# jl6017/AutoURDF

Hardware: AMD Instinct MI355X
Metric: registered frames/sec (N=4096 pts, K=20 clusters) (higher is better)
Workload: dtype f32

## Files before the change

autourdf_amd/csrc/train_backward.hip:

```cpp
#include <cmath>
#include <cstddef>
#include <cstring>
#include "train_dev.h"

namespace creg {

__device__ __forceinline__ TrainState advance_state(const TrainState& S, float loss, const Hyper& hy, double bc1, float bc2_sqrt) {
    TrainState N = S;
    const bool improved = loss < S.min_loss;
    N.last_loss = loss;
    N.epochs_run = S.epochs_run + 1;
    const int count = improved ? 0 : S.count + 1;
    N.min_loss = improved ? loss : S.min_loss;
    N.best_epoch = improved ? S.epochs_run : S.best_epoch;
    N.count = count;
    N.stopped = (!improved && count > hy.stop) ? 1 : S.stopped;
    if (!N.stopped) {
        N.step = S.step + 1;
        N.step_size = (float)(S.lr / bc1);
        N.bc2_sqrt = bc2_sqrt;
        const double cur = (double)loss;
        if (cur < S.sched_best * (1.0 - 1e-4)) { N.sched_best = cur; N.sched_bad = 0; }
        else N.sched_bad = S.sched_bad + 1;
        if (N.sched_bad > hy.patience) {
            const double nl = fmax(S.lr * (double)hy.factor, 0.0);
            if (S.lr - nl > 1e-8) N.lr = nl;
            N.sched_bad = 0;
        }
    }
    return N;
}

constexpr int GC_QMAX = 3;
__device__ __forceinline__ void gradc_role(const Dims& D, const Ws& W, int epoch, int nbx, int nby, int k) {
    __shared__ float red[4][14];
    __shared__ float s_loss;
    __shared__ float s_go[16];
    const int tid = threadIdx.x, lane = tid & 63, wv = tid >> 6;
    const TrainState S = W.state[epoch & 1];
    const int b0 = W.off[k], e0 = W.off[k + 1];
    const Hyper hy = *W.hyper;
    float a = tid < nbx ? W.lossp_x[tid] : 0.f, b = tid < nby ? W.lossp_y[tid] : 0.f;
    const float m2v = W.m2[16 * k + (tid & 15)];
    float sv[16];
#pragma unroll
    for (int i = 0; i < 16; ++i) sv[i] = W.head_save[16 * k + i];
    const float* h2cur = (epoch & 1) ? W.h2[1] : W.h2[0];
    float w3v[GC_QMAX][8], h2v[GC_QMAX];
#pragma unroll
    for (int q = 0; q < GC_QMAX; ++q) {
        const int o = min(q * 256 + tid, D.H2 - 1);
        const bool isA = o < D.HA;
        const float* Pc = (epoch & 1) ? W.P1 : W.P;
        const float* wb = isA ? Pc + D.oW3A + o : Pc + D.oW3B + (o - D.HA);
        const int stride = isA ? D.HA : D.HB, nj = isA ? D.OA : D.OB;
#pragma unroll
        for (int j = 0; j < 8; ++j) w3v[q][j] = wb[(size_t)min(j, nj - 1) * stride];
        h2v[q] = h2cur[(size_t)k * D.H2 + o];
    }
    asm volatile("" :: "v"(a), "v"(b), "v"(m2v), "v"(sv[0]), "v"(sv[1]), "v"(sv[2]), "v"(sv[3]), "v"(sv[4]), "v"(sv[5]), "v"(sv[6]), "v"(sv[7]),
                 "v"(sv[8]), "v"(sv[9]), "v"(sv[10]), "v"(sv[11]), "v"(sv[12]), "v"(sv[13]), "v"(sv[14]), "v"(sv[15]), "v"(b0), "v"(e0), "v"(hy.lr));
#pragma unroll
    for (int q = 0; q < GC_QMAX; ++q)
        asm volatile("" :: "v"(h2v[q]), "v"(w3v[q][0]), "v"(w3v[q][1]), "v"(w3v[q][2]), "v"(w3v[q][3]), "v"(w3v[q][4]), "v"(w3v[q][5]), "v"(w3v[q][6]),
                     "v"(w3v[q][7]));
    if (S.stopped) {
        if (k == 0 && tid == 0) {
            TrainState E = S; E.stopped = 1;
            W.state[(epoch + 1) & 1] = E;
        }
        return;
    }
    const int n_first = min(b0 + tid, D.NP - 1);
    const float4 p_first = W.pts4[n_first];
    const int4 c_first = W.cnt4[n_first];
    const int s_first = W.sgn_x[n_first];
    const float4 pr_first = W.pred4[n_first];
    for (int i = tid + 256; i < nbx; i += 256) a += W.lossp_x[i];
    for (int i = tid + 256; i < nby; i += 256) b += W.lossp_y[i];
    a = wave_sum_fast(a); b = wave_sum_fast(b);
    if (lane == 0) { red[wv][0] = a; red[wv][1] = b; }
    __syncthreads();
    if (tid == 0) {
        const float sa = ((red[0][0] + red[1][0]) + red[2][0]) + red[3][0];
        const float sb = ((red[0][1] + red[1][1]) + red[2][1]) + red[3][1];
        s_loss = sa / (float)D.NP + sb / (float)D.NT;
    }
    __syncthreads();
    const float loss = s_loss;
    TrainState N = advance_state(S, loss, hy, S.next_bc1, S.next_bc2s);
    const bool improved = loss < S.min_loss;
    if (improved) {
        for (int n = b0 + tid; n < e0; n += 256) {
            const float4 p = (n == b0 + tid) ? pr_first : W.pred4[n];
            W.best_pred[3 * (size_t)n] = p.x; W.best_pred[3 * (size_t)n + 1] = p.y; W.best_pred[3 * (size_t)n + 2] = p.z;
        }
        if (tid < 16) W.best_m[16 * k + tid] = m2v;
    }
    if (k == 0 && tid == 0) {
        N.next_bc1 = W.bc1[min(N.step + 1, D.epochs)];
        N.next_bc2s = W.bc2s[min(N.step + 1, D.epochs)];
        W.state[(epoch + 1) & 1] = N;
        W.loss_hist[S.epochs_run] = loss;
        W.lr_hist[S.epochs_run] = (float)S.lr;
        W.result[0] = N.min_loss; W.result[1] = (float)N.epochs_run; W.result[2] = (float)N.lr; W.result[3] = (float)N.best_epoch;
    }
    if (N.stopped) return;
    const float gx = 1.0f / (float)D.NP, gy = 1.0f / (float)D.NT;
    float acc[12];
#pragma unroll
    for (int i = 0; i < 12; ++i) acc[i] = 0.f;
    for (int n = b0 + tid; n < e0; n += 256) {
        const bool first = n == b0 + tid;
        const float4 p = first ? p_first : W.pts4[n];
        const int4 c = first ? c_first : W.cnt4[n];
        const int sb = first ? s_first : W.sgn_x[n];
        const float g[3] = {((sb & 1) ? gx : -gx) + gy * (float)c.x, ((sb & 2) ? gx : -gx) + gy * (float)c.y,
                            ((sb & 4) ? gx : -gx) + gy * (float)c.z};
#pragma unroll
        for (int q = 0; q < 3; ++q) {
            acc[4 * q] = fmaf(g[q], p.x, acc[4 * q]); acc[4 * q + 1] = fmaf(g[q], p.y, acc[4 * q + 1]);
            acc[4 * q + 2] = fmaf(g[q], p.z, acc[4 * q + 2]); acc[4 * q + 3] += g[q];
        }
    }
    __syncthreads();
#pragma unroll
    for (int i = 0; i < 12; ++i) { const float r = wave_sum_fast(acc[i]); if (lane == 0) red[wv][i] = r; }
    __syncthreads();
    if (tid == 0) {
        float G12[12];
        for (int i = 0; i < 12; ++i) G12[i] = ((red[0][i] + red[1][i]) + red[2][i]) + red[3][i];
        for (int i = 0; i < 16; ++i) W.gm2[16 * k + i] = i < 12 ? G12[i] : 0.f;
        const float G[9] = {G12[0], G12[1], G12[2], G12[4], G12[5], G12[6], G12[8], G12[9], G12[10]};
        const float gt[3] = {G12[3], G12[7], G12[11]};
        float go[16];
        for (int i = 0; i < 16; ++i) go[i] = 0.f;
        if (D.rot == ROT_6D) {
            go[0] = gt[0]; go[1] = gt[1]; go[2] = gt[2];
            rot6d_to_matrix_vjp(sv, G, go + 4);
        } else if (D.rot == ROT_RPY) {
            go[0] = gt[0]; go[1] = gt[1]; go[2] = gt[2];
            float ge[3];
            euler_xyz_to_matrix_vjp(sv, G, ge);
            for (int i = 0; i < 3; ++i) go[4 + i] = ge[i] * (1.f - sv[4 + i] * sv[4 + i]);
        } else if (D.rot == ROT_Q) {
            go[0] = gt[0]; go[1] = gt[1]; go[2] = gt[2];
            float gu[4];
            quat_to_matrix_vjp(sv, G, gu);
            const float nrm = sv[4];
            if (nrm > 1e-12f) {
                const float dot = sv[0] * gu[0] + sv[1] * gu[1] + sv[2] * gu[2] + sv[3] * gu[3];
#pragma unroll
                for (int i = 0; i < 4; ++i) go[4 + i] = (gu[i] - sv[i] * dot) / nrm;
            } else {
#pragma unroll
                for (int i = 0; i < 4; ++i) go[4 + i] = gu[i] / 1e-12f;
            }
        } else {
            float gdq[8];
            dq_to_se3_vjp(sv, G, gt, gdq);
            for (int i = 0; i < 8; ++i) go[4 + i] = gdq[i];
        }
        for (int i = 0; i < 12; ++i) { W.g_out[16 * k + i] = go[i]; s_go[i] = go[i]; }
    }
    __syncthreads();
#pragma unroll
    for (int q = 0; q < GC_QMAX; ++q) {
        const int o = q * 256 + tid;
        if (o < D.H2) {
            const bool isA = o < D.HA;
            const int nj = isA ? D.OA : D.OB, gofs = isA ? 0 : 4;
            float sum = 0.f;
#pragma unroll
            for (int j = 0; j < 8; ++j) if (j < nj) sum = fmaf(s_go[gofs + j], w3v[q][j], sum);
            W.g_h2[(size_t)k * D.H2 + o] = sum * act_grad(h2v[q], D.slope);
        }
    }
}

__global__ __launch_bounds__(256) void k_gradc(Dims D, Ws W0, int epoch, int nbx, int nby, size_t bstride) {
    asm volatile("" :: "s"(W0.P), "s"(W0.P1), "s"(W0.h2[0]), "s"(W0.h2[1]), "s"(W0.head_save), "s"(W0.m2), "s"(W0.gm2), "s"(W0.pts4), "s"(W0.pred4),
                 "s"(W0.sgn_x), "s"(W0.cnt4), "s"(W0.lossp_x), "s"(W0.lossp_y), "s"(W0.g_out), "s"(W0.g_h2), "s"(W0.state), "s"(W0.bc1), "s"(W0.bc2s),
                 "s"(W0.best_m), "s"(W0.best_pred), "s"(W0.loss_hist), "s"(W0.lr_hist), "s"(W0.result), "s"(W0.off), "s"(W0.hyper),
                 "s"(D.rot), "s"(D.K), "s"(D.H2), "s"(D.HA), "s"(D.HB), "s"(D.OA), "s"(D.OB), "s"(D.NP), "s"(D.NT), "s"(D.epochs), "s"(D.slope),
                 "s"(D.oW3A), "s"(D.oW3B), "s"(epoch), "s"(nbx), "s"(nby), "s"(bstride));
    const Ws W = ws_shift(W0, blockIdx.z * bstride);
    gradc_role(D, W, epoch, nbx, nby, blockIdx.x);
}

__device__ __forceinline__ float adam_value(float p, float& mm, float& vv, float g, float step_size, float bc2_sqrt) {
    const float b1w = (float)(1.0 - 0.9), b2 = 0.999f, b2w = (float)(1.0 - 0.999);
    mm = mm + b1w * (g - mm);
    vv = vv * b2 + (b2w * g) * g;
    const float denom = sqrtf(vv) / bc2_sqrt + 1e-8f;
    return p + (-step_size * mm) / denom;
}

#ifdef CREG_BD_STAMPS
struct BdStamps {
    unsigned long long first[256], endB[256], endD[256], startB[256], startD[256];
    unsigned long long phase[2][8], blocks[2];
    int armed;
};
__device__ BdStamps g_bd_st;
#endif
constexpr int BD_THREADS = 512;
constexpr int B2_THREADS = BD_THREADS;
constexpr int B2_WAVES = B2_THREADS / 64;
constexpr int B2_CB = 16;
constexpr int B2_RB = 32;
__host__ __device__ inline int b2_smem_floats(int K, int IN, int H2) {
    return B2_WAVES * B2_RB * B2_CB + K * IN + 2 * K * B2_CB + H2 * B2_CB;
}
__device__ __forceinline__ float row_sum16(float v) {
    CREG_DPP_STEP(v, 0xB1, 0xF);
    CREG_DPP_STEP(v, 0x4E, 0xF);
    CREG_DPP_STEP(v, 0x141, 0xF);
    CREG_DPP_STEP(v, 0x140, 0xF);
    return v;
}

template <int KW, bool X>
__device__ __forceinline__ void bwd2_role(const Dims& D, const Ws& W, int epoch, int blk, float* sh, unsigned long long bd_entry) {
    constexpr int NS = KW / 4;
    constexpr bool V4 = KW % 16 == 0;
    constexpr int NA = V4 ? NS / 4 : NS;
    float* red = sh;
    float* encs = red + B2_WAVES * B2_RB * B2_CB;
    float* gxs = encs + D.K * D.IN;
    float* xt = gxs + D.K * B2_CB;
    float* w2s = xt + D.K * B2_CB;
    const int tid = threadIdx.x, lane = tid & 63, wv = tid >> 6, lj = lane & 15, kk = lane >> 4;
    __builtin_amdgcn_s_waitcnt(0x0F70);
    const int c0 = blk * B2_CB, par = epoch & 1;
    const float* x1cur = par ? W.x1[1] : W.x1[0];
    float* x1next = par ? W.x1[0] : W.x1[1];
    const float* Pc = par ? W.P1 : W.P;
    float* Pn = par ? W.P : W.P1;
    BD_T0
    {
        const float* src = Pc + D.oW2 + (size_t)(wv * KW + (lane >> 2)) * D.H + c0 + 4 * (lane & 3);
        float* dst = w2s + wv * KW * B2_CB;
#pragma unroll
        for (int i = 0; i < KW; i += 16)
            if (i + (lane >> 2) < KW)
                __builtin_amdgcn_global_load_lds((const __attribute__((address_space(1))) void*)(src + (size_t)i * D.H),
                                                 (__attribute__((address_space(3))) void*)(dst + i * B2_CB), 16, 0, 0);
    }
    const float* gbase = W.g_h2 + wv * KW + (V4 ? 4 * kk : kk);
    auto load_a = [&](int row, float* dst) {
        const float* g = gbase + (size_t)min(row, D.K - 1) * D.H2;
#pragma unroll
        for (int q = 0; q < NA; ++q) {
            if constexpr (V4) { const float4 v = *(const float4*)(g + 16 * q); dst[4 * q] = v.x; dst[4 * q + 1] = v.y; dst[4 * q + 2] = v.z; dst[4 * q + 3] = v.w; }
            else dst[q] = g[4 * q];
        }
    };
    float a0[NS], a1[NS];
    const bool two0 = D.K > 16;
    load_a(lj, a0);
    if (two0) load_a(16 + lj, a1);
    const int half = tid >> 8, t2 = tid & 255, row = t2 >> 4, i4 = t2 & 15, hu = c0 + row;
    const bool ain = 4 * i4 < D.IN;
    const int ei = min(4 * i4, D.IN - 4);
    const size_t wi = (size_t)D.oW1 + (size_t)hu * D.IN + ei;
    float4 pw = *(const float4*)(Pc + wi), pm = *(const float4*)(W.AM + wi), pv = *(const float4*)(W.AV + wi);
    const bool ain2 = X && 64 + 4 * i4 < D.IN;
    const int ei2 = min(64 + 4 * i4, D.IN - 4);
    const size_t wi2 = (size_t)D.oW1 + (size_t)hu * D.IN + ei2;
    float4 pw2, pm2, pv2;
    if constexpr (X) { pw2 = *(const float4*)(Pc + wi2); pm2 = *(const float4*)(W.AM + wi2); pv2 = *(const float4*)(W.AV + wi2); }
    float pb = Pc[D.ob1 + hu], mb = W.AM[D.ob1 + hu], vb = W.AV[D.ob1 + hu];
    float xv0 = x1cur[(size_t)min(tid >> 4, D.K - 1) * D.H + c0 + (tid & 15)];
    {
        const int n = D.K * D.IN / 4;
        constexpr int NPC = 8;
#pragma unroll
        for (int c = 0; c < NPC; ++c) {
            const int i = c * B2_THREADS + tid;
            if (i < n)
                __builtin_amdgcn_global_load_lds((const __attribute__((address_space(1))) void*)((const float4*)W.enc + i),
                                                 (__attribute__((address_space(3))) void*)((float4*)encs + c * B2_THREADS + (tid & ~63)), 16, 0, 0);
        }
    }
    __builtin_amdgcn_sched_barrier(0);
    const TrainState S = W.state[(epoch + 1) & 1];
    const bool live = !S.stopped;
    __builtin_amdgcn_sched_barrier(0);
    BD_T
    stage_wait();
    float wb[NS];
#pragma unroll
    for (int s = 0; s < NS; ++s) {
        const int o = V4 ? 16 * (s >> 2) + 4 * kk + (s & 3) : 4 * s + kk;
        wb[s] = w2s[(wv * KW + o) * B2_CB + lj];
    }
    for (int r0 = 0; r0 < D.K; r0 += B2_RB) {
        const int nr = min(B2_RB, D.K - r0);
        const bool two = nr > 16;
        float xv = xv0;
        if (r0) {
            load_a(r0 + lj, a0);
            if (two) load_a(r0 + 16 + lj, a1);
            xv = x1cur[(size_t)min(r0 + (tid >> 4), D.K - 1) * D.H + c0 + (tid & 15)];
        }
        f32x4 acc0 = {0.f, 0.f, 0.f, 0.f}, acc1 = {0.f, 0.f, 0.f, 0.f};
        if (two) {
#pragma unroll
            for (int s = 0; s < NS; ++s) {
                acc0 = __builtin_amdgcn_mfma_f32_16x16x4f32(a0[s], wb[s], acc0, 0, 0, 0);
                acc1 = __builtin_amdgcn_mfma_f32_16x16x4f32(a1[s], wb[s], acc1, 0, 0, 0);
            }
        } else {
#pragma unroll
            for (int s = 0; s < NS; ++s) acc0 = __builtin_amdgcn_mfma_f32_16x16x4f32(a0[s], wb[s], acc0, 0, 0, 0);
        }
        if (r0) __syncthreads();
        {
            float* o = red + (wv * B2_RB + 4 * kk) * B2_CB + lj;
#pragma unroll
            for (int v = 0; v < 4; ++v) { o[v * B2_CB] = acc0[v]; if (two) o[(16 + v) * B2_CB] = acc1[v]; }
        }
        stage_wait();
        __syncthreads();
        if (r0 == 0) { BD_T }
        if (!live) return;
        if (tid < nr * B2_CB) {
            float sum = red[tid];
#pragma unroll
            for (int w2 = 1; w2 < B2_WAVES; ++w2) sum += red[w2 * B2_RB * B2_CB + tid];
            gxs[r0 * B2_CB + tid] = sum * act_grad(xv, D.slope);
        }
    }
    __syncthreads();
    BD_T
    float4 ag = make_float4(0.f, 0.f, 0.f, 0.f), ag2 = make_float4(0.f, 0.f, 0.f, 0.f);
    float gsum = 0.f;
    for (int r = 0; r < D.K; ++r) {
        const float g = gxs[r * B2_CB + row];
        const float4 e = *(const float4*)(encs + r * D.IN + ei);
        ag.x = fmaf(g, e.x, ag.x); ag.y = fmaf(g, e.y, ag.y); ag.z = fmaf(g, e.z, ag.z); ag.w = fmaf(g, e.w, ag.w);
        if constexpr (X) {
            const float4 e2 = *(const float4*)(encs + r * D.IN + ei2);
            ag2.x = fmaf(g, e2.x, ag2.x); ag2.y = fmaf(g, e2.y, ag2.y); ag2.z = fmaf(g, e2.z, ag2.z); ag2.w = fmaf(g, e2.w, ag2.w);
        }
        gsum += g;
    }
    float4 nw;
    nw.x = adam_value(pw.x, pm.x, pv.x, ag.x, S.step_size, S.bc2_sqrt);
    nw.y = adam_value(pw.y, pm.y, pv.y, ag.y, S.step_size, S.bc2_sqrt);
    nw.z = adam_value(pw.z, pm.z, pv.z, ag.z, S.step_size, S.bc2_sqrt);
    nw.w = adam_value(pw.w, pm.w, pv.w, ag.w, S.step_size, S.bc2_sqrt);
    float4 nw2 = make_float4(0.f, 0.f, 0.f, 0.f);
    if constexpr (X) {
        nw2.x = adam_value(pw2.x, pm2.x, pv2.x, ag2.x, S.step_size, S.bc2_sqrt);
        nw2.y = adam_value(pw2.y, pm2.y, pv2.y, ag2.y, S.step_size, S.bc2_sqrt);
        nw2.z = adam_value(pw2.z, pm2.z, pv2.z, ag2.z, S.step_size, S.bc2_sqrt);
        nw2.w = adam_value(pw2.w, pm2.w, pv2.w, ag2.w, S.step_size, S.bc2_sqrt);
    }
    pb = adam_value(pb, mb, vb, gsum, S.step_size, S.bc2_sqrt);
    if (live && half == 0) {
        if (ain) { st4_wt(Pn, wi, nw); st4_wt(W.AM, wi, pm); st4_wt(W.AV, wi, pv); }
        if constexpr (X) if (ain2) { st4_wt(Pn, wi2, nw2); st4_wt(W.AM, wi2, pm2); st4_wt(W.AV, wi2, pv2); }
        if (i4 == 0) { Pn[D.ob1 + hu] = pb; W.AM[D.ob1 + hu] = mb; W.AV[D.ob1 + hu] = vb; }
    }
    BD_T
    for (int r = half; r < D.K; r += 2) {
        const float4 e = *(const float4*)(encs + r * D.IN + ei);
        float v = ain ? fmaf(nw.w, e.w, fmaf(nw.z, e.z, fmaf(nw.y, e.y, nw.x * e.x))) : 0.f;
        if constexpr (X) {
            const float4 e2 = *(const float4*)(encs + r * D.IN + ei2);
            if (ain2) v = fmaf(nw2.w, e2.w, fmaf(nw2.z, e2.z, fmaf(nw2.y, e2.y, fmaf(nw2.x, e2.x, v))));
        }
        v = row_sum16(v) + pb;
        if (i4 == 0) xt[r * B2_CB + row] = act_f(v, D.slope);
    }
    __syncthreads();
    if (live)
        for (int t = tid; t < D.K * (B2_CB / 2); t += B2_THREADS) {
            const int r = t >> 3, c2 = 2 * (t & 7);
            *(nn_f2*)(x1next + (size_t)r * D.H + c0 + c2) = nn_f2{xt[r * B2_CB + c2], xt[r * B2_CB + c2 + 1]};
        }
    BD_TEND(0, epoch);
}


constexpr int DW_UNITS = 16;
constexpr int DW_TILES = 4;
constexpr int DW_KC = 5;
__host__ __device__ inline int dw_blocks(const Dims& D) { return D.H2 / DW_UNITS + 2; }

__device__ __forceinline__ void dw_role(const Dims& D, const Ws& W, int epoch, int blk, unsigned long long bd_entry) {
    const int lane = threadIdx.x & 63, wv = threadIdx.x >> 6, lj = lane & 15, q = lane >> 4;
    __builtin_amdgcn_s_waitcnt(0x0F70);
    const int par = epoch & 1;
    const float* Pc = par ? W.P1 : W.P;
    float* Pn = par ? W.P : W.P1;
    const float* x1cur = par ? W.x1[1] : W.x1[0];
    const float* h2cur = par ? W.h2[1] : W.h2[0];
    asm volatile("" : "+s"(x1cur), "+s"(h2cur));
    const int nb2 = D.H2 / DW_UNITS;
    int u0, nu, n_in, oW, ob, astride, gstride;
    const float *amat, *gmat;
    if (blk < nb2) { u0 = blk * DW_UNITS; nu = DW_UNITS; n_in = D.H; oW = D.oW2 + u0 * D.H; ob = D.ob2 + u0; amat = x1cur; astride = D.H; gmat = W.g_h2 + u0; gstride = D.H2; }
    else if (blk == nb2) { u0 = 0; nu = D.OA; n_in = D.HA; oW = D.oW3A; ob = D.ob3A; amat = h2cur; astride = D.H2; gmat = W.g_out; gstride = 16; }
    else { u0 = 0; nu = D.OB; n_in = D.HB; oW = D.oW3B; ob = D.ob3B; amat = h2cur + D.HA; astride = D.H2; gmat = W.g_out + 4; gstride = 16; }
    if (nu == 0) return;
    if (64 * wv >= n_in) return;
    BD_T0
    const int unit = min(lj, nu - 1);
    const bool ulive = lj < nu;
    const int i0 = 64 * wv;
    const int po = (oW + unit * n_in + i0 + 4 * q) * 4;
    const __amdgpu_buffer_rsrc_t rP = buf_rsrc(Pc, D.NPAR * 4), rM = buf_rsrc(W.AM, D.NPAR * 4), rV = buf_rsrc(W.AV, D.NPAR * 4);
    f32x4 acc[DW_TILES];
#pragma unroll
    for (int t = 0; t < DW_TILES; ++t) acc[t] = f32x4{0.f, 0.f, 0.f, 0.f};
    float gb = 0.f;
    const __amdgpu_buffer_rsrc_t rA = buf_rsrc(amat, (D.KP * astride - (int)(amat - (blk < nb2 ? x1cur : h2cur))) * 4);
    const __amdgpu_buffer_rsrc_t rG = buf_rsrc(gmat, (D.KP * gstride - (blk < nb2 ? u0 : (blk == nb2 ? 0 : 4))) * 4);
    const int aoff = (q * astride + i0 + 16 * (lj & 3) + 4 * (lj >> 2)) * 4, goff = (q * gstride + unit) * 4;
    float bop[DW_KC];
    float4 aop[DW_KC];
    auto load_ops = [&](int s0) {
#pragma unroll
        for (int s = 0; s < DW_KC; ++s) {
            const int r4 = 4 * (s0 + s);
            bop[s] = __uint_as_float(__builtin_amdgcn_raw_buffer_load_b32(rG, goff, r4 * gstride * 4, 0));
            aop[s] = ld_buf4(rA, aoff, r4 * astride * 4);
        }
    };
    auto mfma_ops = [&]() {
#pragma unroll
        for (int s = 0; s < DW_KC; ++s) {
            acc[0] = __builtin_amdgcn_mfma_f32_16x16x4f32(aop[s].x, bop[s], acc[0], 0, 0, 0);
            acc[1] = __builtin_amdgcn_mfma_f32_16x16x4f32(aop[s].y, bop[s], acc[1], 0, 0, 0);
            acc[2] = __builtin_amdgcn_mfma_f32_16x16x4f32(aop[s].z, bop[s], acc[2], 0, 0, 0);
            acc[3] = __builtin_amdgcn_mfma_f32_16x16x4f32(aop[s].w, bop[s], acc[3], 0, 0, 0);
        }
#pragma unroll
        for (int s = 0; s < DW_KC; ++s) gb += bop[s];
    };
    load_ops(0);
    __builtin_amdgcn_sched_barrier(0);
    const TrainState S = W.state[(epoch + 1) & 1];
    float pb = Pc[ob + unit], mb = W.AM[ob + unit], vb = W.AV[ob + unit];
    __builtin_amdgcn_sched_barrier(0);
    float4 pw[DW_TILES], pm[DW_TILES], pv[DW_TILES];
    bool vl[DW_TILES];
#pragma unroll
    for (int v = 0; v < DW_TILES; ++v) {
        vl[v] = ulive && i0 + 16 * v + 4 * q < n_in;
        pw[v] = ld_buf4(rP, po + 64 * v, 0); pm[v] = ld_buf4(rM, po + 64 * v, 0); pv[v] = ld_buf4(rV, po + 64 * v, 0);
        __builtin_amdgcn_sched_barrier(0);
    }
    BD_T
    mfma_ops();
    for (int s0 = DW_KC; 4 * s0 < D.KP; s0 += DW_KC) {
        load_ops(s0);
        __builtin_amdgcn_sched_barrier(0);
        mfma_ops();
    }
    BD_T
    if (S.stopped) return;
#pragma unroll
    for (int v = 0; v < DW_TILES; ++v) {
        float4 nw;
        nw.x = adam_value(pw[v].x, pm[v].x, pv[v].x, acc[0][v], S.step_size, S.bc2_sqrt);
        nw.y = adam_value(pw[v].y, pm[v].y, pv[v].y, acc[1][v], S.step_size, S.bc2_sqrt);
        nw.z = adam_value(pw[v].z, pm[v].z, pv[v].z, acc[2][v], S.step_size, S.bc2_sqrt);
        nw.w = adam_value(pw[v].w, pm[v].w, pv[v].w, acc[3][v], S.step_size, S.bc2_sqrt);
        if (vl[v]) { const int e = po / 4 + 16 * v; st4_wt(Pn, e, nw); st4_wt(W.AM, e, pm[v]); st4_wt(W.AV, e, pv[v]); }
    }
    if (wv == 0) {
        float sum = gb;
        sum += __shfl_xor(gb, 16, 64);
        sum += __shfl_xor(sum, 32, 64);
        pb = adam_value(pb, mb, vb, sum, S.step_size, S.bc2_sqrt);
        if (q == 0 && ulive) { Pn[ob + unit] = pb; W.AM[ob + unit] = mb; W.AV[ob + unit] = vb; }
    }
    BD_TEND(1, epoch);
}

template <int NC, int KW, bool X = false>
__global__ __launch_bounds__(BD_THREADS, 4) void k_bd(Dims D, Ws W0, int epoch, size_t bstride, int nz) {
    extern __shared__ __attribute__((aligned(16))) char smem[];
#ifdef CREG_BD_STAMPS
    const unsigned long long bd_entry = wall_clock64();
#else
    const unsigned long long bd_entry = 0;
#endif
#ifndef CREG_BD_NO_TOUCH
    asm volatile("" :: "s"(W0.P), "s"(W0.P1), "s"(W0.AM), "s"(W0.AV), "s"(W0.enc), "s"(W0.x1[0]), "s"(W0.x1[1]), "s"(W0.h2[0]), "s"(W0.h2[1]),
                 "s"(W0.g_out), "s"(W0.g_h2), "s"(W0.state), "s"(D.K), "s"(D.KP), "s"(D.IN), "s"(D.H), "s"(D.H2), "s"(D.HA), "s"(D.HB), "s"(D.OA),
                 "s"(D.OB), "s"(D.oW1), "s"(D.ob1), "s"(D.oW2), "s"(D.ob2), "s"(D.oW3A), "s"(D.ob3A), "s"(D.oW3B), "s"(D.ob3B), "s"(D.NPAR),
                 "s"(D.slope), "s"(epoch), "s"(bstride), "s"(nz));
#endif
    const int nB = D.H / B2_CB, nD = dw_blocks(D);
    int i = blockIdx.x;
    const bool roleB = i < nB * nz;
    if (!roleB) i -= nB * nz;
    const int n = roleB ? nB : nD, z = i / n, blk = i - z * n;
    const Ws W = ws_shift(W0, (size_t)z * bstride);
#ifdef CREG_BD_ONLY
    if ((CREG_BD_ONLY == 1) != roleB) return;
#endif
    if (roleB) bwd2_role<KW, X>(D, W, epoch, blk, (float*)smem, bd_entry);
    else dw_role(D, W, epoch, blk, bd_entry);
}
constexpr int BD_K_MAX_6D_512 = 193;
constexpr int BD_LDS_MAX = 160 * 1024;
static int bd_lds_bytes(const Dims& D) { return (int)sizeof(float) * b2_smem_floats(D.K, D.IN, D.H2); }
bool backward_fits(const Dims& D) {
    if (D.rot == ROT_6D && D.H == 512 && D.K > BD_K_MAX_6D_512) return false;
    return D.K * D.IN / 4 <= 8 * BD_THREADS && bd_lds_bytes(D) <= BD_LDS_MAX && D.H2 % 32 == 0 && D.H % B2_CB == 0 && D.H2 <= 256 * GC_QMAX;
}
void launch_gradc(const Dims& D, const Slice& S, size_t bstride, int epoch, hipStream_t s) {
    hipLaunchKernelGGL(k_gradc, dim3(D.K, 1, S.nz), dim3(256), 0, s, D, S.W, epoch, D.nbx, D.nby, bstride);
}
template <typename F>
static void by_bd(const Dims& D, F f) {
    by_nc(D.H, [&](auto nc) {
        constexpr int NC = decltype(nc)::value;
        if (D.IN > 64) f(k_bd<NC, 12 * NC, true>);
        else if (D.HA) f(k_bd<NC, 12 * NC>);
        else f(k_bd<NC, 8 * NC>);
    });
}
int bd_raise_lds(const Dims& D) {
    hipError_t e = hipSuccess;
    by_bd(D, [&](auto kern) { e = hipFuncSetAttribute((const void*)kern, hipFuncAttributeMaxDynamicSharedMemorySize, BD_LDS_MAX); });
    if (e != hipSuccess) {
        set_error("creg_train_plan_create: cannot raise the dynamic LDS limit of k_bd: %s", hipGetErrorString(e));
        return CREG_EHIP;
    }
    return CREG_OK;
}
void launch_bd(const Dims& D, const Slice& S, size_t bstride, int epoch, hipStream_t s) {
    const int per = D.H / B2_CB + dw_blocks(D);
    by_bd(D, [&](auto kern) { hipLaunchKernelGGL(kern, dim3(per * S.nz), dim3(BD_THREADS), bd_lds_bytes(D), s, D, S.W, epoch, bstride, S.nz); });
}

int bd_stamps_arm(bool on) {
#ifdef CREG_BD_STAMPS
    static BdStamps z;
    if (on) {
        memset(&z, 0, sizeof(z)); memset(z.first, 0xff, sizeof(z.first)); memset(z.startB, 0xff, sizeof(z.startB)); memset(z.startD, 0xff, sizeof(z.startD));
        z.armed = 1;
        CREG_HIP(hipMemcpyToSymbol(HIP_SYMBOL(g_bd_st), &z, sizeof(z)));
    } else {
        z.armed = 0;
        CREG_HIP(hipMemcpyToSymbol(HIP_SYMBOL(g_bd_st), &z.armed, sizeof(int), offsetof(BdStamps, armed)));
    }
#endif
    return CREG_OK;
}

}
using namespace creg;

#ifdef CREG_BD_STAMPS
extern "C" int creg_debug_bd_stamps(double* out) {
    BdStamps* z = new BdStamps;
    if (hipMemcpyFromSymbol(z, HIP_SYMBOL(g_bd_st), sizeof(*z)) != hipSuccess) { delete z; return CREG_EHIP; }
    for (int i = 0; i < 24; ++i) out[i] = 0.0;
    int n = 0;
    for (int sl = 0; sl < 256; ++sl) {
        if (z->first[sl] == ~0ull || !z->endB[sl] || !z->endD[sl]) continue;
        ++n;
        const double f = (double)z->first[sl];
        out[0] += ((double)(z->endB[sl] > z->endD[sl] ? z->endB[sl] : z->endD[sl]) - f) / 100.0;
        out[1] += ((double)z->startB[sl] - f) / 100.0; out[2] += ((double)z->endB[sl] - f) / 100.0;
        out[3] += ((double)z->startD[sl] - f) / 100.0; out[4] += ((double)z->endD[sl] - f) / 100.0;
    }
    for (int i = 0; i < 5; ++i) out[i] /= n ? n : 1;
    out[5] = n ? (double)z->blocks[0] / n : 0; out[6] = n ? (double)z->blocks[1] / n : 0; out[7] = n;
    for (int r = 0; r < 2; ++r)
        for (int k = 0; k < 8; ++k) out[8 + 8 * r + k] = z->blocks[r] ? (double)z->phase[r][k] / (double)z->blocks[r] / 100.0 : 0.0;
    delete z;
    return CREG_OK;
}
#endif
```

Before: 166.7.

## Batch LDS loads in backward weight-update loops and remap column blocks across XCDs

```diff
diff --git a/autourdf_amd/csrc/train_backward.hip b/autourdf_amd/csrc/train_backward.hip
--- a/autourdf_amd/csrc/train_backward.hip
+++ b/autourdf_amd/csrc/train_backward.hip
@@ -1,6 +1,7 @@
 #include <cmath>
 #include <cstddef>
 #include <cstring>
+#include <type_traits>
 #include "train_dev.h"
 
 namespace creg {
@@ -209,6 +210,10 @@
 constexpr int B2_WAVES = B2_THREADS / 64;
 constexpr int B2_CB = 16;
 constexpr int B2_RB = 32;
+constexpr int B2_NB = 5;
+#ifndef CREG_BD_PAIR_XCD
+#define CREG_BD_PAIR_XCD 1
+#endif
 __host__ __device__ inline int b2_smem_floats(int K, int IN, int H2) {
     return B2_WAVES * B2_RB * B2_CB + K * IN + 2 * K * B2_CB + H2 * B2_CB;
 }
@@ -232,7 +237,9 @@
     float* w2s = xt + D.K * B2_CB;
     const int tid = threadIdx.x, lane = tid & 63, wv = tid >> 6, lj = lane & 15, kk = lane >> 4;
     __builtin_amdgcn_s_waitcnt(0x0F70);
-    const int c0 = blk * B2_CB, par = epoch & 1;
+    const int nB = D.H / B2_CB;
+    const int cb = CREG_BD_PAIR_XCD && nB % 16 == 0 ? (blk & 7) * (nB >> 3) + (blk >> 3) : blk;
+    const int c0 = cb * B2_CB, par = epoch & 1;
     const float* x1cur = par ? W.x1[1] : W.x1[0];
     float* x1next = par ? W.x1[0] : W.x1[1];
     const float* Pc = par ? W.P1 : W.P;
@@ -336,15 +343,34 @@
     BD_T
     float4 ag = make_float4(0.f, 0.f, 0.f, 0.f), ag2 = make_float4(0.f, 0.f, 0.f, 0.f);
     float gsum = 0.f;
-    for (int r = 0; r < D.K; ++r) {
-        const float g = gxs[r * B2_CB + row];
-        const float4 e = *(const float4*)(encs + r * D.IN + ei);
-        ag.x = fmaf(g, e.x, ag.x); ag.y = fmaf(g, e.y, ag.y); ag.z = fmaf(g, e.z, ag.z); ag.w = fmaf(g, e.w, ag.w);
-        if constexpr (X) {
-            const float4 e2 = *(const float4*)(encs + r * D.IN + ei2);
-            ag2.x = fmaf(g, e2.x, ag2.x); ag2.y = fmaf(g, e2.y, ag2.y); ag2.z = fmaf(g, e2.z, ag2.z); ag2.w = fmaf(g, e2.w, ag2.w);
-        }
-        gsum += g;
+    auto dw1_batch = [&](int r0, auto guarded) {
+        float g[B2_NB];
+        float4 e[B2_NB], e2[B2_NB];
+#pragma unroll
+        for (int j = 0; j < B2_NB; ++j) {
+            const int r = decltype(guarded)::value ? min(r0 + j, D.K - 1) : r0 + j;
+            g[j] = gxs[r * B2_CB + row];
+            e[j] = *(const float4*)(encs + r * D.IN + ei);
+            if constexpr (X) e2[j] = *(const float4*)(encs + r * D.IN + ei2);
+        }
+        static_assert(B2_NB == 5, "the operand lists below name five rows");
+        asm volatile("" : "+v"(g[0]), "+v"(g[1]), "+v"(g[2]), "+v"(g[3]), "+v"(g[4]), "+v"(e[0].x), "+v"(e[1].x), "+v"(e[2].x), "+v"(e[3].x), "+v"(e[4].x));
+        if constexpr (X) asm volatile("" : "+v"(e2[0].x), "+v"(e2[1].x), "+v"(e2[2].x), "+v"(e2[3].x), "+v"(e2[4].x));
+        __builtin_amdgcn_sched_barrier(0);
+#pragma unroll
+        for (int j = 0; j < B2_NB; ++j) {
+            if (decltype(guarded)::value && r0 + j >= D.K) continue;
+            ag.x = fmaf(g[j], e[j].x, ag.x); ag.y = fmaf(g[j], e[j].y, ag.y); ag.z = fmaf(g[j], e[j].z, ag.z); ag.w = fmaf(g[j], e[j].w, ag.w);
+            if constexpr (X) {
+                ag2.x = fmaf(g[j], e2[j].x, ag2.x); ag2.y = fmaf(g[j], e2[j].y, ag2.y); ag2.z = fmaf(g[j], e2[j].z, ag2.z); ag2.w = fmaf(g[j], e2[j].w, ag2.w);
+            }
+            gsum += g[j];
+        }
+    };
+    {
+        int r0 = 0;
+        for (; r0 + B2_NB <= D.K; r0 += B2_NB) dw1_batch(r0, std::false_type{});
+        if (r0 < D.K) dw1_batch(r0, std::true_type{});
     }
     float4 nw;
     nw.x = adam_value(pw.x, pm.x, pv.x, ag.x, S.step_size, S.bc2_sqrt);
@@ -365,15 +391,42 @@
         if (i4 == 0) { Pn[D.ob1 + hu] = pb; W.AM[D.ob1 + hu] = mb; W.AV[D.ob1 + hu] = vb; }
     }
     BD_T
-    for (int r = half; r < D.K; r += 2) {
-        const float4 e = *(const float4*)(encs + r * D.IN + ei);
-        float v = ain ? fmaf(nw.w, e.w, fmaf(nw.z, e.z, fmaf(nw.y, e.y, nw.x * e.x))) : 0.f;
-        if constexpr (X) {
-            const float4 e2 = *(const float4*)(encs + r * D.IN + ei2);
-            if (ain2) v = fmaf(nw2.w, e2.w, fmaf(nw2.z, e2.z, fmaf(nw2.y, e2.y, fmaf(nw2.x, e2.x, v))));
-        }
-        v = row_sum16(v) + pb;
-        if (i4 == 0) xt[r * B2_CB + row] = act_f(v, D.slope);
+    auto act_batch = [&](int rb, auto guarded) {
+        float4 e[B2_NB], e2[B2_NB];
+        float v[B2_NB];
+#pragma unroll
+        for (int j = 0; j < B2_NB; ++j) {
+            const int r = decltype(guarded)::value ? min(rb + 2 * j, D.K - 1) : rb + 2 * j;
+            e[j] = *(const float4*)(encs + r * D.IN + ei);
+            if constexpr (X) e2[j] = *(const float4*)(encs + r * D.IN + ei2);
+        }
+        asm volatile("" : "+v"(e[0].x), "+v"(e[1].x), "+v"(e[2].x), "+v"(e[3].x), "+v"(e[4].x));
+        if constexpr (X) asm volatile("" : "+v"(e2[0].x), "+v"(e2[1].x), "+v"(e2[2].x), "+v"(e2[3].x), "+v"(e2[4].x));
+        __builtin_amdgcn_sched_barrier(0);
+#pragma unroll
+        for (int j = 0; j < B2_NB; ++j) {
+            v[j] = ain ? fmaf(nw.w, e[j].w, fmaf(nw.z, e[j].z, fmaf(nw.y, e[j].y, nw.x * e[j].x))) : 0.f;
+            if constexpr (X)
+                if (ain2) v[j] = fmaf(nw2.w, e2[j].w, fmaf(nw2.z, e2[j].z, fmaf(nw2.y, e2[j].y, fmaf(nw2.x, e2[j].x, v[j]))));
+        }
+#pragma unroll
+        for (int j = 0; j < B2_NB; ++j) CREG_DPP_STEP(v[j], 0xB1, 0xF);
+#pragma unroll
+        for (int j = 0; j < B2_NB; ++j) CREG_DPP_STEP(v[j], 0x4E, 0xF);
+#pragma unroll
+        for (int j = 0; j < B2_NB; ++j) CREG_DPP_STEP(v[j], 0x141, 0xF);
+#pragma unroll
+        for (int j = 0; j < B2_NB; ++j) CREG_DPP_STEP(v[j], 0x140, 0xF);
+        if (i4 == 0) {
+#pragma unroll
+            for (int j = 0; j < B2_NB; ++j)
+                if (!decltype(guarded)::value || rb + 2 * j < D.K) xt[(rb + 2 * j) * B2_CB + row] = act_f(v[j] + pb, D.slope);
+        }
+    };
+    {
+        int rb = half;
+        for (; rb + 2 * (B2_NB - 1) < D.K; rb += 2 * B2_NB) act_batch(rb, std::false_type{});
+        if (rb < D.K) act_batch(rb, std::true_type{});
     }
     __syncthreads();
     if (live)
```

Result: no change. 166.6 (-0.1%).
